# zhang-xuan1314/ABC-Net

Measured on AMD Instinct MI355X. Metric: training images/sec (384x384, b16/GPU), higher is better.
Workload: dtype bf16; 1 GPU; unet.py train step (pack+fwd+fused loss+bwd+allreduce+Adam), 384x384, batch 16/GPU, dropout 0.2; global_batch=16, parallelism=dp1, graph=True, device_meters=False, device_rasteriser=False, device_extraction=False, logits_stored=True

## Files before the change

### abc-net_amd/csrc/bn_act.hip

```cpp
#include "common.hpp"
#include "../../include/abcnet_hip.h"
#include "capi_util.hpp"
#include "reduce_bn.hpp"
#include <stdlib.h>

namespace {

__device__ inline void bn_finalize_fwd_body(const abc_bn_fwd_desc& d, int pstride) {
    __shared__ double sm[4];
    const int c = blockIdx.x;
    if (c >= d.C) return;
    const int rows = d.rows == 4 ? 4 : 2;
    double s1 = 0.0, s2 = 0.0;
    for (int k = threadIdx.x; k < d.nblk; k += 256) {
        s1 += (double)d.partial[((size_t)k * rows + 0) * pstride + c];
        s2 += (double)d.partial[((size_t)k * rows + 1) * pstride + c];
    }
    s1 = block_sum_f64(s1, sm);
    s2 = block_sum_f64(s2, sm);
    if (threadIdx.x == 0) {
        const double mean = s1 / d.count;
        double var = s2 / d.count - mean * mean;
        if (var < 0.0) var = 0.0;
        const float invstd = (float)(1.0 / sqrt(var + (double)d.eps));
        const float sc = d.gamma[c] * invstd;
        d.scale[c] = sc;
        d.shift[c] = d.beta[c] - (float)mean * sc;
        d.mean[c] = (float)mean;
        d.invstd[c] = invstd;
        if (d.running_mean != nullptr) {
            const double unb = d.count > 1.0 ? var * d.count / (d.count - 1.0) : var;
            d.running_mean[c] = (1.f - d.momentum) * d.running_mean[c] + d.momentum * (float)mean;
            d.running_var[c] = (1.f - d.momentum) * d.running_var[c] + d.momentum * (float)unb;
            if (c == 0 && d.num_batches_tracked != nullptr) *d.num_batches_tracked += 1;
        }
    }
}

__global__ __launch_bounds__(256) void bn_finalize_fwd_kernel(const abc_bn_fwd_desc d) { bn_finalize_fwd_body(d, d.C); }
constexpr int MAX_BNB = 8;
struct BnFwdBatch { abc_bn_fwd_desc d[MAX_BNB]; int pstride; };
__global__ __launch_bounds__(256) void bn_finalize_fwd_batch_kernel(const BnFwdBatch bt) {
    bn_finalize_fwd_body(bt.d[blockIdx.y], bt.pstride > 0 ? bt.pstride : bt.d[blockIdx.y].C);
}

__global__ void bn_eval_kernel(const float* gamma, const float* beta, const float* rm, const float* rv, float* scale,
                               float* shift, int C, float eps) {
    const int c = blockIdx.x * blockDim.x + threadIdx.x;
    if (c >= C) return;
    const float sc = gamma[c] / sqrtf(rv[c] + eps);
    scale[c] = sc;
    shift[c] = beta[c] - rm[c] * sc;
}

__global__ void bn_eval_fold_kernel(const float* gamma, const float* beta, const float* rm, const float* rv, const float* cb, float* scale,
                                    float* bias_out, int C, float eps) {
    const int c = blockIdx.x * blockDim.x + threadIdx.x;
    if (c >= C) return;
    const float sc = gamma[c] / sqrtf(rv[c] + eps);
    scale[c] = sc;
    bias_out[c] = ((cb ? cb[c] : 0.f) - rm[c]) * sc + beta[c];
}

__global__ __launch_bounds__(256) void bn_finalize_bwd_kernel(const abc_bn_bwd_desc d) { bn_finalize_bwd_body(d, d.C, blockIdx.x); }
struct BnBwdBatch { abc_bn_bwd_desc d[MAX_BNB]; int pstride; };
__global__ __launch_bounds__(256) void bn_finalize_bwd_batch_kernel(const BnBwdBatch bt) {
    bn_finalize_bwd_body(bt.d[blockIdx.y], bt.pstride > 0 ? bt.pstride : bt.d[blockIdx.y].C, blockIdx.x);
}

template <typename T> struct VecOf;
template <> struct VecOf<float> { static constexpr int N = 4; };
template <> struct VecOf<bf16> { static constexpr int N = 8; };

template <typename T, int N> __device__ inline void ldv(const T* p, float* v) { LoadVec<T, N>::ld(p, v); }
template <int N> __device__ inline void stv(float* p, const float* v) {
    f32x4 t; t[0] = v[0]; t[1] = v[1]; t[2] = v[2]; t[3] = v[3];
    *(f32x4*)p = t;
}
template <int N> __device__ inline void stv(bf16* p, const float* v) {
    bf16x8 t;
#pragma unroll
    for (int j = 0; j < 8; ++j) t[j] = (bf16)v[j];
    *(bf16x8*)p = t;
}

template <typename T>
__global__ __launch_bounds__(256) void act_bwd_plain_kernel(const abc_act_bwd_desc d) {
    constexpr int N = VecOf<T>::N;
    __shared__ float red[256][2 * N + 1];
    const int ncv = d.C / N;
    const unsigned nitems = (unsigned)((int64_t)d.B * d.H * d.W * ncv);
    const unsigned stride = gridDim.x * 256u;
    const int tid = threadIdx.x;
    const int cv = (int)((blockIdx.x * 256 + tid) % ncv);
    const int c = cv * N;
    const int lg = 31 - __builtin_clz((unsigned)ncv);
    float sc[N], sh[N], sl[N], mu[N];
#pragma unroll
    for (int j = 0; j < N; ++j) { sc[j] = d.scale[c + j]; sh[j] = d.shift[c + j]; sl[j] = d.slope[c + j]; mu[j] = d.mean[c + j]; }
    float a1[N], a2[N];
#pragma unroll
    for (int j = 0; j < N; ++j) { a1[j] = 0.f; a2[j] = 0.f; }
    const T* yr = (const T*)d.y_raw + d.cy_off + c;
    const T* ds = (const T*)d.dA_same + d.csame_off + c;
    T* g = (T*)d.g + c;
    auto one = [&](const float* x, const float* da, size_t p) {
        float out[N];
#pragma unroll
        for (int j = 0; j < N; ++j) {
            const float y = fmaf(x[j], sc[j], sh[j]);
            const float gg = y > 0.f ? da[j] : sl[j] * da[j];
            out[j] = gg;
            a1[j] += gg;
            a2[j] = fmaf(gg, x[j] - mu[j], a2[j]);
        }
        stv<N>(g + p * d.ld_g, out);
    };
    unsigned it = blockIdx.x * 256u + tid;
    for (; it + stride < nitems; it += 2 * stride) {
        const size_t p0 = it >> lg, p1 = (it + stride) >> lg;
        float x0[N], d0[N], x1[N], d1[N];
        ldv<T, N>(yr + p0 * d.ld_y, x0); ldv<T, N>(ds + p0 * d.ld_same, d0);
        ldv<T, N>(yr + p1 * d.ld_y, x1); ldv<T, N>(ds + p1 * d.ld_same, d1);
        one(x0, d0, p0);
        one(x1, d1, p1);
    }
    if (it < nitems) {
        const size_t p0 = it >> lg;
        float x0[N], d0[N];
        ldv<T, N>(yr + p0 * d.ld_y, x0); ldv<T, N>(ds + p0 * d.ld_same, d0);
        one(x0, d0, p0);
    }
#pragma unroll
    for (int j = 0; j < N; ++j) { red[tid][j] = a1[j]; red[tid][N + j] = a2[j]; }
    __syncthreads();
    for (int cc = tid; cc < d.C; cc += 256) {
        const int v = cc / N, j = cc % N;
        float s1 = 0.f, s2 = 0.f;
        for (int t = v; t < 256; t += ncv) { s1 += red[t][j]; s2 += red[t][N + j]; }
        d.partial[((size_t)blockIdx.x * 2 + 0) * d.C + cc] = s1;
        d.partial[((size_t)blockIdx.x * 2 + 1) * d.C + cc] = s2 * d.invstd[cc];
    }
}

template <typename T>
__global__ __launch_bounds__(256) void act_bwd_kernel(const abc_act_bwd_desc d) {
    constexpr int N = VecOf<T>::N;
    __shared__ float red[256][2 * N + 1];
    const int ncv = d.C / N;
    const bool pooled = d.dA_pool != nullptr;
    const int Hw = pooled ? d.H / 2 : d.H, Ww = pooled ? d.W / 2 : d.W;
    const int64_t nitems = (int64_t)d.B * Hw * Ww * ncv;
    const int64_t stride = (int64_t)gridDim.x * 256;
    const int tid = threadIdx.x;
    const int cv = (int)((blockIdx.x * 256 + tid) % ncv);
    const int c = cv * N;
    float sc[N], sh[N], sl[N], mu[N], is[N];
#pragma unroll
    for (int j = 0; j < N; ++j) {
        sc[j] = d.scale[c + j]; sh[j] = d.shift[c + j]; sl[j] = d.slope[c + j]; mu[j] = d.mean[c + j]; is[j] = d.invstd[c + j];
    }
    float a1[N], a2[N];
#pragma unroll
    for (int j = 0; j < N; ++j) { a1[j] = 0.f; a2[j] = 0.f; }
    const T* yr = (const T*)d.y_raw;
    const T* ds = (const T*)d.dA_same;
    const T* dp = (const T*)d.dA_pool;
    T* g = (T*)d.g;
    const float dscale = d.drop_p > 0.f ? 1.f / (1.f - d.drop_p) : 1.f;
    const uint32_t dseed = d.drop_seed + ((d.drop_p > 0.f && d.drop_salt) ? *d.drop_salt : 0u);

    const bool pow2 = (ncv & (ncv - 1)) == 0;
    const int lg = 31 - __builtin_clz((unsigned)ncv);
    const unsigned n32 = (unsigned)nitems, st32 = (unsigned)stride;
    for (unsigned it = blockIdx.x * 256u + tid; it < n32; it += st32) {
        unsigned pix = pow2 ? (it >> lg) : (it / (unsigned)ncv);
        if (!pooled) {
            const size_t p = pix;
            float x[N], da[N], out[N];
            ldv<T, N>(yr + p * d.ld_y + d.cy_off + c, x);
            ldv<T, N>(ds + p * d.ld_same + d.csame_off + c, da);
#pragma unroll
            for (int j = 0; j < N; ++j) {
                const float y = fmaf(x[j], sc[j], sh[j]);
                float gg = da[j] * (y > 0.f ? 1.f : sl[j]);
                if (d.drop_p > 0.f)
                    gg = abc_drop_keep((uint32_t)(p * d.drop_ld + d.cy_off + c + j), dseed, d.drop_p) ? gg * dscale : 0.f;
                out[j] = gg;
                a1[j] += gg;
                a2[j] += gg * ((x[j] - mu[j]) * is[j]);
            }
            stv<N>(g + p * d.ld_g + c, out);
        } else {
            const int wx = (int)(pix % (unsigned)Ww); pix /= (unsigned)Ww;
            const int wy = (int)(pix % (unsigned)Hw);
            const int b = (int)(pix / (unsigned)Hw);
            float x[4][N], dpool[N];
            size_t pq[4];
#pragma unroll
            for (int q = 0; q < 4; ++q) {
                pq[q] = ((size_t)b * d.H + 2 * wy + (q >> 1)) * d.W + 2 * wx + (q & 1);
                ldv<T, N>(yr + pq[q] * d.ld_y + d.cy_off + c, x[q]);
            }
            ldv<T, N>(dp + (((size_t)b * Hw + wy) * Ww + wx) * d.ld_pool + d.cpool_off + c, dpool);
            int arg[N];
            float yv[4][N];
#pragma unroll
            for (int j = 0; j < N; ++j) {
                float best = 0.f;
                arg[j] = 0;
#pragma unroll
                for (int q = 0; q < 4; ++q) {
                    const float y = fmaf(x[q][j], sc[j], sh[j]);
                    yv[q][j] = y;
                    const float av = fmaxf(y, sl[j] * y);
                    if (q == 0 || av > best) { best = av; arg[j] = q; }
                }
            }
#pragma unroll
            for (int q = 0; q < 4; ++q) {
                float da[N], out[N];
                if (ds != nullptr) ldv<T, N>(ds + pq[q] * d.ld_same + d.csame_off + c, da);
#pragma unroll
                for (int j = 0; j < N; ++j) {
                    float up = (arg[j] == q) ? dpool[j] : 0.f;
                    if (ds != nullptr) up += da[j];
                    const float gg = up * (yv[q][j] > 0.f ? 1.f : sl[j]);
                    out[j] = gg;
                    a1[j] += gg;
                    a2[j] += gg * ((x[q][j] - mu[j]) * is[j]);
                }
                stv<N>(g + pq[q] * d.ld_g + c, out);
            }
        }
    }
    if (pooled && ((d.H | d.W) & 1)) {
        const int wodd = d.W & 1, hodd = d.H & 1;
        const int ncol = wodd ? d.H : 0;
        const int nrow = hodd ? 2 * Ww : 0;
        const unsigned nl = (unsigned)(ncol + nrow);
        const unsigned n2 = (unsigned)d.B * nl * (unsigned)ncv;
        for (unsigned it = blockIdx.x * 256u + tid; it < n2; it += st32) {
            unsigned l = pow2 ? (it >> lg) : (it / (unsigned)ncv);
            const int b = (int)(l / nl);
            l -= (unsigned)b * nl;
            const int y = (int)l < ncol ? (int)l : d.H - 1, x = (int)l < ncol ? d.W - 1 : (int)l - ncol;
            const size_t p = ((size_t)b * d.H + y) * d.W + x;
            float xv[N], da[N], out[N];
            ldv<T, N>(yr + p * d.ld_y + d.cy_off + c, xv);
            if (ds != nullptr) ldv<T, N>(ds + p * d.ld_same + d.csame_off + c, da);
#pragma unroll
            for (int j = 0; j < N; ++j) {
                const float yv = fmaf(xv[j], sc[j], sh[j]);
                const float gg = (ds != nullptr ? da[j] : 0.f) * (yv > 0.f ? 1.f : sl[j]);
                out[j] = gg;
                a1[j] += gg;
                a2[j] += gg * ((xv[j] - mu[j]) * is[j]);
            }
            stv<N>(g + p * d.ld_g + c, out);
        }
    }
#pragma unroll
    for (int j = 0; j < N; ++j) { red[tid][j] = a1[j]; red[tid][N + j] = a2[j]; }
    __syncthreads();
    for (int cc = tid; cc < d.C; cc += 256) {
        const int v = cc / N, j = cc % N;
        float s1 = 0.f, s2 = 0.f;
        for (int t = v; t < 256; t += ncv) { s1 += red[t][j]; s2 += red[t][N + j]; }
        d.partial[((size_t)blockIdx.x * 2 + 0) * d.C + cc] = s1;
        d.partial[((size_t)blockIdx.x * 2 + 1) * d.C + cc] = s2;
    }
}

template <typename T>
__global__ __launch_bounds__(256) void bn_apply_kernel(const abc_bn_apply_desc d) {
    constexpr int N = VecOf<T>::N;
    const int ncv = d.C / N;
    const int64_t nitems = d.npix * ncv;
    const int64_t stride = (int64_t)gridDim.x * 256;
    T* g = (T*)d.g;
    T* o = d.out ? (T*)d.out : g;
    const int ld_o = d.out ? d.ld_out : d.ld_g;
    const T* yr = (const T*)d.y_raw;
    for (int64_t it = (int64_t)blockIdx.x * 256 + threadIdx.x; it < nitems; it += stride) {
        const int64_t p = it / ncv;
        const int c = (int)(it % ncv) * N;
        float gv[N], x[N], out[N];
        ldv<T, N>(g + p * d.ld_g + c, gv);
        ldv<T, N>(yr + p * d.ld_y + d.cy_off + c, x);
#pragma unroll
        for (int j = 0; j < N; ++j) {
            const float xh = (x[j] - d.mean[c + j]) * d.invstd[c + j];
            out[j] = d.gscale[c + j] * (gv[j] - d.k1[c + j] - xh * d.k2[c + j]);
        }
        stv<N>(o + p * ld_o + c, out);
    }
}
// ... 84 lines not shown
    const T* base = x + c_off + cv * N;
    int64_t p = (int64_t)blockIdx.x * PL + pl;
    const int64_t step = (int64_t)gridDim.x * PL;
    for (; p + 3 * step < npix; p += 4 * step) {
        float a[4][N], wv[4];
#pragma unroll
        for (int u = 0; u < 4; ++u) { ldv<T, N>(base + (p + u * step) * ld, a[u]); wv[u] = w[p + u * step]; }
#pragma unroll
        for (int u = 0; u < 4; ++u)
#pragma unroll
            for (int j = 0; j < N; ++j) { acc[j] += a[u][j]; accw[j] = fmaf(a[u][j], wv[u], accw[j]); }
    }
    for (; p < npix; p += step) {
        float a[N];
        ldv<T, N>(base + p * ld, a);
        const float wv = w[p];
#pragma unroll
        for (int j = 0; j < N; ++j) { acc[j] += a[j]; accw[j] = fmaf(a[j], wv, accw[j]); }
    }
#pragma unroll
    for (int j = 0; j < N; ++j) { red[threadIdx.x][j] = acc[j]; red[threadIdx.x][N + j] = accw[j]; }
    __syncthreads();
    for (int c = threadIdx.x; c < 2 * C; c += 256) {
        const int row = c / C, cc = c - row * C;
        const int v = cc / N, j = cc % N;
        float s = 0.f;
        for (int q = 0; q < PL; ++q) s += red[q * ncv + v][row * N + j];
        work[((size_t)blockIdx.x * 2 + row) * C + cc] = s;
    }
}
__global__ __launch_bounds__(256) void colsum_w1_reduce_kernel(const float* work, int nblk, int C, float* out_sum, float* out_w) {
    __shared__ double sm[4];
    const int c = blockIdx.x, row = blockIdx.y;
    double s = 0.0;
    for (int k = threadIdx.x; k < nblk; k += 256) s += (double)work[((size_t)k * 2 + row) * C + c];
    s = block_sum_f64(s, sm);
    if (threadIdx.x == 0) {
        if (row == 0) { if (out_sum != nullptr) out_sum[c] = (float)s; }
        else out_w[c] = (float)s;
    }
}

__global__ void fill_kernel(float* p, float v, int64_t n) {
    for (int64_t i = (int64_t)blockIdx.x * blockDim.x + threadIdx.x; i < n; i += (int64_t)gridDim.x * blockDim.x) p[i] = v;
}

__global__ __launch_bounds__(256) void nhwc_to_nchw_kernel(const float* src, int ld, int c_off, int C, int HW, float* dst) {
    __shared__ float tile[32][33];
    const int b = blockIdx.z;
    const int p0 = blockIdx.x * 32, c0 = blockIdx.y * 32;
    const int tx = threadIdx.x & 31, ty = threadIdx.x >> 5;
    for (int k = ty; k < 32; k += 8) {
        const int p = p0 + k, c = c0 + tx;
        tile[k][tx] = (p < HW && c < C) ? src[((size_t)b * HW + p) * ld + c_off + c] : 0.f;
    }
    __syncthreads();
    for (int k = ty; k < 32; k += 8) {
        const int c = c0 + k, p = p0 + tx;
        if (p < HW && c < C) dst[((size_t)b * C + c) * HW + p] = tile[tx][k];
    }
}
__global__ __launch_bounds__(256) void nchw_to_nhwc_kernel(const float* src, int C, int HW, float* dst, int ld, int c_off) {
    __shared__ float tile[32][33];
    const int b = blockIdx.z;
    const int p0 = blockIdx.x * 32, c0 = blockIdx.y * 32;
    const int tx = threadIdx.x & 31, ty = threadIdx.x >> 5;
    for (int k = ty; k < 32; k += 8) {
        const int c = c0 + k, p = p0 + tx;
        tile[k][tx] = (p < HW && c < C) ? src[((size_t)b * C + c) * HW + p] : 0.f;
    }
    __syncthreads();
    for (int k = ty; k < 32; k += 8) {
        const int p = p0 + k, c = c0 + tx;
        if (p < HW && c < C) dst[((size_t)b * HW + p) * ld + c_off + c] = tile[tx][k];
    }
}

static int ew_blocks(int64_t nitems) {
    int64_t b = (nitems + 255) / 256;
    if (b > 2048) b = 2048;
    if (b < 1) b = 1;
    return (int)b;
}

}

extern "C" int abc_bn_finalize_fwd(const abc_bn_fwd_desc* d, abc_stream_t stream) {
    if (d->C < 1 || d->nblk < 1) return abc_fail(ABC_EINVAL, "bn_finalize_fwd: empty");
    hipLaunchKernelGGL(bn_finalize_fwd_kernel, dim3(d->C), dim3(256), 0, (hipStream_t)stream, *d);
    return abc_check_launch("bn_finalize_fwd");
}

extern "C" int abc_bn_finalize_fwd_batch(const abc_bn_fwd_desc* descs, int32_t n, int32_t pstride, abc_stream_t stream) {
    if (n < 1 || n > MAX_BNB) return abc_fail(ABC_EINVAL, "bn_finalize_fwd_batch: 1..8 layers");
    BnFwdBatch bt;
    int cmax = 0;
    for (int i = 0; i < n; ++i) { bt.d[i] = descs[i]; cmax = descs[i].C > cmax ? descs[i].C : cmax; if (descs[i].C < 1 || descs[i].nblk < 1) return abc_fail(ABC_EINVAL, "bn_finalize_fwd_batch: empty"); }
    for (int i = n; i < MAX_BNB; ++i) bt.d[i] = descs[0];
    bt.pstride = pstride;
    hipLaunchKernelGGL(bn_finalize_fwd_batch_kernel, dim3(cmax, n), dim3(256), 0, (hipStream_t)stream, bt);
    return abc_check_launch("bn_finalize_fwd_batch");
}

extern "C" int abc_bn_finalize_bwd_batch(const abc_bn_bwd_desc* descs, int32_t n, int32_t pstride, abc_stream_t stream) {
    if (n < 1 || n > MAX_BNB) return abc_fail(ABC_EINVAL, "bn_finalize_bwd_batch: 1..8 layers");
    BnBwdBatch bt;
    int cmax = 0;
    for (int i = 0; i < n; ++i) { bt.d[i] = descs[i]; cmax = descs[i].C > cmax ? descs[i].C : cmax; if (descs[i].C < 1 || descs[i].nblk < 1) return abc_fail(ABC_EINVAL, "bn_finalize_bwd_batch: empty"); }
    for (int i = n; i < MAX_BNB; ++i) bt.d[i] = descs[0];
    bt.pstride = pstride;
    hipLaunchKernelGGL(bn_finalize_bwd_batch_kernel, dim3(cmax, n), dim3(256), 0, (hipStream_t)stream, bt);
    return abc_check_launch("bn_finalize_bwd_batch");
}

extern "C" int abc_bn_eval_coeffs(const float* gamma, const float* beta, const float* running_mean, const float* running_var,
                                  float* scale, float* shift, int32_t C, float eps, abc_stream_t stream) {
    hipLaunchKernelGGL(bn_eval_kernel, dim3(abc_cdiv(C, 256)), dim3(256), 0, (hipStream_t)stream, gamma, beta, running_mean,
                       running_var, scale, shift, C, eps);
    return abc_check_launch("bn_eval_coeffs");
}

extern "C" int abc_bn_eval_fold(const float* gamma, const float* beta, const float* running_mean, const float* running_var,
                                const float* conv_bias, float* scale, float* bias_out, int32_t C, float eps, abc_stream_t stream) {
    hipLaunchKernelGGL(bn_eval_fold_kernel, dim3(abc_cdiv(C, 256)), dim3(256), 0, (hipStream_t)stream, gamma, beta, running_mean,
                       running_var, conv_bias, scale, bias_out, C, eps);
    return abc_check_launch("bn_eval_fold");
}

extern "C" int abc_bn_finalize_bwd(const abc_bn_bwd_desc* d, abc_stream_t stream) {
    if (d->C < 1 || d->nblk < 1) return abc_fail(ABC_EINVAL, "bn_finalize_bwd: empty");
    hipLaunchKernelGGL(bn_finalize_bwd_kernel, dim3(d->C), dim3(256), 0, (hipStream_t)stream, *d);
    return abc_check_launch("bn_finalize_bwd");
}

static int act_bwd_check(const abc_act_bwd_desc* d) {
    const int N = d->dtype == ABC_BF16 ? 8 : 4;
    if (d->C % N) return abc_fail(ABC_EINVAL, "act_bwd: C must be a multiple of the vector width");
    const int ncv = d->C / N;
    if (ncv > 256 || (256 % ncv)) return abc_fail(ABC_EUNSUPPORTED, "act_bwd: C/vec must divide 256");
    if (d->dA_pool && (((d->H | d->W) & 1) && d->drop_p > 0.f)) return abc_fail(ABC_EUNSUPPORTED, "act_bwd: odd pooled dims with dropout");
    if (!d->dA_pool && !d->dA_same) return abc_fail(ABC_EINVAL, "act_bwd: no gradient source");
    if ((d->ld_y | d->ld_g | d->cy_off) % N) return abc_fail(ABC_EINVAL, "act_bwd: alignment");
    if ((int64_t)d->B * d->H * d->W * ncv >= (int64_t(1) << 31)) return abc_fail(ABC_EUNSUPPORTED, "act_bwd: tensor too large for 32-bit indexing");
    return ABC_OK;
}

extern "C" int abc_act_bwd_blocks(const abc_act_bwd_desc* d) {
    const int N = d->dtype == ABC_BF16 ? 8 : 4;
    const bool pooled = d->dA_pool != nullptr;
    const int64_t n = (int64_t)d->B * (pooled ? d->H / 2 : d->H) * (pooled ? d->W / 2 : d->W) * (d->C / N);
    return ew_blocks(n);
}

extern "C" int abc_act_bwd(const abc_act_bwd_desc* d, abc_stream_t stream) {
    int rc = act_bwd_check(d);
    if (rc) return rc;
    const int nb = abc_act_bwd_blocks(d);
    if (d->dA_pool == nullptr && d->drop_p <= 0.f) {
        if (d->dtype == ABC_BF16) hipLaunchKernelGGL(act_bwd_plain_kernel<bf16>, dim3(nb), dim3(256), 0, (hipStream_t)stream, *d);
        else hipLaunchKernelGGL(act_bwd_plain_kernel<float>, dim3(nb), dim3(256), 0, (hipStream_t)stream, *d);
        return abc_check_launch("act_bwd");
    }
    if (d->dtype == ABC_BF16) hipLaunchKernelGGL(act_bwd_kernel<bf16>, dim3(nb), dim3(256), 0, (hipStream_t)stream, *d);
    else hipLaunchKernelGGL(act_bwd_kernel<float>, dim3(nb), dim3(256), 0, (hipStream_t)stream, *d);
    return abc_check_launch("act_bwd");
}

extern "C" int abc_bn_apply_bwd(const abc_bn_apply_desc* d, abc_stream_t stream) {
    const int N = d->dtype == ABC_BF16 ? 8 : 4;
    if (d->C % N || (d->ld_g | d->ld_y | d->cy_off) % N || (d->out && d->ld_out % N)) return abc_fail(ABC_EINVAL, "bn_apply: alignment");
    const int nb = ew_blocks(d->npix * (d->C / N));
    if (d->dtype == ABC_BF16) hipLaunchKernelGGL(bn_apply_kernel<bf16>, dim3(nb), dim3(256), 0, (hipStream_t)stream, *d);
    else hipLaunchKernelGGL(bn_apply_kernel<float>, dim3(nb), dim3(256), 0, (hipStream_t)stream, *d);
    return abc_check_launch("bn_apply_bwd");
}

extern "C" int abc_colsum_blocks(int64_t npix) {
    int64_t b = (npix + 63) / 64;
    return (int)(b < 1 ? 1 : (b > 1024 ? 1024 : b));
}

extern "C" int abc_colsum(const void* x, int32_t dtype, int64_t npix, int32_t ld, int32_t c_off, int32_t C,
                          const float* chan_scale, float* work, float* out, abc_stream_t stream) {
    const int nb = abc_colsum_blocks(npix);
    hipStream_t st = (hipStream_t)stream;
    if (C > 512) return abc_fail(ABC_EUNSUPPORTED, "colsum: C > 512");
    {
        const int N = dtype == ABC_BF16 ? 8 : 4;
        const int ncv = C / N;
        if (C % N == 0 && ncv >= 1 && ncv <= 256 && 256 % ncv == 0 && ld % N == 0 && c_off % N == 0) {
            if (dtype == ABC_BF16)
                hipLaunchKernelGGL(colsum_vec_kernel<bf16>, dim3(nb), dim3(256), 0, st, (const bf16*)x, npix, ld, c_off, C, chan_scale, work);
            else
                hipLaunchKernelGGL(colsum_vec_kernel<float>, dim3(nb), dim3(256), 0, st, (const float*)x, npix, ld, c_off, C, chan_scale, work);
            hipLaunchKernelGGL(colsum_reduce_kernel, dim3(C), dim3(256), 0, st, (const float*)work, nb, C, out);
            return abc_check_launch("colsum");
        }
    }
    int CW = 1;
    while (CW < C && CW < 64) CW <<= 1;
    if (dtype == ABC_BF16)
        hipLaunchKernelGGL(colsum_kernel<bf16>, dim3(nb), dim3(256), 0, st, (const bf16*)x, npix, ld, c_off, C, chan_scale, work, CW);
    else
        hipLaunchKernelGGL(colsum_kernel<float>, dim3(nb), dim3(256), 0, st, (const float*)x, npix, ld, c_off, C, chan_scale, work, CW);
    hipLaunchKernelGGL(colsum_reduce_kernel, dim3(C), dim3(256), 0, st, (const float*)work, nb, C, out);
    return abc_check_launch("colsum");
}

extern "C" int abc_colsum_w1(const void* x, int32_t dtype, int64_t npix, int32_t ld, int32_t c_off, int32_t C, const float* w,
                             float* work, float* out_sum, float* out_w, abc_stream_t stream) {
    const int nb = abc_colsum_blocks(npix);
    const int N = dtype == ABC_BF16 ? 8 : 4;
    const int ncv = C / N;
    if (x == nullptr || w == nullptr || work == nullptr || out_w == nullptr) return abc_fail(ABC_EINVAL, "colsum_w1: x, w, work and out_w are required");
    if (C % N || ncv < 1 || ncv > 256 || 256 % ncv || ld % N || c_off % N)
        return abc_fail(ABC_EUNSUPPORTED, "colsum_w1: C / vector width must divide 256, ld and c_off be multiples of the vector width");
    hipStream_t st = (hipStream_t)stream;
    if (dtype == ABC_BF16) hipLaunchKernelGGL(colsum_w1_kernel<bf16>, dim3(nb), dim3(256), 0, st, (const bf16*)x, npix, ld, c_off, C, w, work);
    else hipLaunchKernelGGL(colsum_w1_kernel<float>, dim3(nb), dim3(256), 0, st, (const float*)x, npix, ld, c_off, C, w, work);
    hipLaunchKernelGGL(colsum_w1_reduce_kernel, dim3(C, 2), dim3(256), 0, st, (const float*)work, nb, C, out_sum, out_w);
    return abc_check_launch("colsum_w1");
}

template <typename InT, typename OutT>
__global__ __launch_bounds__(256) void pool_act_kernel(const InT* x, const float* sc, const float* sh, const float* sl, int Hx, int Wx,
                                                        int ldx, int c_off, int C, int64_t nseg, OutT* out, int ld_out) {
    const int64_t i = (int64_t)blockIdx.x * 256 + threadIdx.x;
    if (i >= nseg) return;
    const int segs = C / 8;
    const int sg = (int)(i % segs);
    int64_t pix = i / segs;
    const int Wo = Wx / 2, Ho = Hx / 2;
    const int xo = (int)(pix % Wo); pix /= Wo;
    const int yo = (int)(pix % Ho);
    const int b = (int)(pix / Ho);
    const int c = c_off + sg * 8;
    float a[8], s_[8], t_[8];
    const bool tr = sc != nullptr;
#pragma unroll
    for (int j = 0; j < 8; ++j) { a[j] = tr ? sc[c + j] : 1.f; s_[j] = tr ? sh[c + j] : 0.f; t_[j] = tr ? sl[c + j] : 1.f; }
    float m[8];
#pragma unroll
    for (int q = 0; q < 4; ++q) {
        float v[8];
        LoadVec<InT, 8>::ld(x + ((size_t)(b * Hx + 2 * yo + (q >> 1)) * Wx + 2 * xo + (q & 1)) * ldx + c, v);
#pragma unroll
        for (int j = 0; j < 8; ++j) {
            const float y = tr ? abc_act(v[j], a[j], s_[j], t_[j]) : v[j];
            m[j] = (q == 0) ? y : fmaxf(m[j], y);
        }
    }
    OutT* dst = out + ((size_t)(b * Ho + yo) * Wo + xo) * ld_out + sg * 8;
    if constexpr (sizeof(OutT) == 2) {
        *(bf16x8*)dst = pack_frag<bf16>(m);
    } else {
        f32x4 lo, hi;
#pragma unroll
        for (int j = 0; j < 4; ++j) { lo[j] = m[j]; hi[j] = m[4 + j]; }
        *(f32x4*)dst = lo; *(f32x4*)(dst + 4) = hi;
    }
}

extern "C" int abc_pool_act(const abc_act_src* src, int32_t dtype_in, int32_t c_off, int32_t C, int32_t B, void* out, int32_t dtype_out,
                            int32_t ld_out, abc_stream_t stream) {
    if (C % 8 || c_off % 8 || src->ldx % 8 || ld_out % 8 || src->Hx < 2 || src->Wx < 2) return abc_fail(ABC_EINVAL, "pool_act: alignment");
    if (src->planar || src->drop_p > 0.f) return abc_fail(ABC_EUNSUPPORTED, "pool_act: planar / dropout source");
    const int64_t nseg = (int64_t)B * (src->Hx / 2) * (src->Wx / 2) * (C / 8);
    const dim3 grid((unsigned)((nseg + 255) / 256));
    hipStream_t st = (hipStream_t)stream;
    if (dtype_in == ABC_BF16 && dtype_out == ABC_BF16)
        hipLaunchKernelGGL((pool_act_kernel<bf16, bf16>), grid, dim3(256), 0, st, (const bf16*)src->x, src->scale, src->shift, src->slope, src->Hx,
                           src->Wx, src->ldx, c_off, C, nseg, (bf16*)out, ld_out);
    else if (dtype_in == ABC_F32 && dtype_out == ABC_F32)
        hipLaunchKernelGGL((pool_act_kernel<float, float>), grid, dim3(256), 0, st, (const float*)src->x, src->scale, src->shift, src->slope,
                           src->Hx, src->Wx, src->ldx, c_off, C, nseg, (float*)out, ld_out);
    else if (dtype_in == ABC_F32 && dtype_out == ABC_BF16)
        hipLaunchKernelGGL((pool_act_kernel<float, bf16>), grid, dim3(256), 0, st, (const float*)src->x, src->scale, src->shift, src->slope,
                           src->Hx, src->Wx, src->ldx, c_off, C, nseg, (bf16*)out, ld_out);
    else return abc_fail(ABC_EUNSUPPORTED, "pool_act: dtype combination");
    return abc_check_launch("pool_act");
}

extern "C" int abc_fill_f32(float* p, float v, int64_t n, abc_stream_t stream) {
    if (n <= 0) return ABC_OK;
    hipLaunchKernelGGL(fill_kernel, dim3(ew_blocks(n)), dim3(256), 0, (hipStream_t)stream, p, v, n);
    return abc_check_launch("fill");
}

extern "C" int abc_nhwc_to_nchw_f32(const float* src, int32_t ld, int32_t c_off, int32_t C, int32_t B, int32_t H, int32_t W,
                                    float* dst, abc_stream_t stream) {
    const int HW = H * W;
    hipLaunchKernelGGL(nhwc_to_nchw_kernel, dim3(abc_cdiv(HW, 32), abc_cdiv(C, 32), B), dim3(256), 0, (hipStream_t)stream, src,
                       ld, c_off, C, HW, dst);
    return abc_check_launch("nhwc_to_nchw");
}

extern "C" int abc_nchw_to_nhwc_f32(const float* src, int32_t C, int32_t B, int32_t H, int32_t W, float* dst, int32_t ld,
                                    int32_t c_off, abc_stream_t stream) {
    const int HW = H * W;
    hipLaunchKernelGGL(nchw_to_nhwc_kernel, dim3(abc_cdiv(HW, 32), abc_cdiv(C, 32), B), dim3(256), 0, (hipStream_t)stream, src,
                       C, HW, dst, ld, c_off);
    return abc_check_launch("nchw_to_nhwc");
}
```

### abc-net_amd/csrc/misc.hip

```cpp
#include "common.hpp"
#include "../../include/abcnet_hip.h"
#include "capi_util.hpp"
#include <string.h>

static thread_local char g_err[256] = "";
int abc_fail(int code, const char* msg) {
    strncpy(g_err, msg, sizeof(g_err) - 1);
    g_err[sizeof(g_err) - 1] = 0;
    return code;
}
int abc_allow_lds(const void* fn, int bytes, unsigned long long* done) {
    int dev = 0;
    if (hipGetDevice(&dev) != hipSuccess) dev = -1;
    if (dev >= 0 && dev < 64 && ((*done >> dev) & 1ull)) return ABC_OK;
    hipError_t e = hipFuncSetAttribute(fn, hipFuncAttributeMaxDynamicSharedMemorySize, bytes);
    if (e != hipSuccess) {
        snprintf(g_err, sizeof(g_err), "hipFuncSetAttribute(MaxDynamicSharedMemorySize=%d) on device %d: %s", bytes, dev, hipGetErrorString(e));
        return ABC_ELAUNCH;
    }
    if (dev >= 0 && dev < 64) *done |= 1ull << dev;
    return ABC_OK;
}
int abc_check_launch(const char* what) {
    hipError_t e = hipGetLastError();
    if (e != hipSuccess) {
        snprintf(g_err, sizeof(g_err), "%s: %s", what, hipGetErrorString(e));
        return ABC_ELAUNCH;
    }
    return ABC_OK;
}
extern "C" const char* abc_last_error(void) { return g_err; }
extern "C" int abc_version(void) { return 101; }
extern "C" int abc_set_reserved_cus(int n) {
    if (n < 0 || n > 128) return abc_fail(ABC_EINVAL, "abc_set_reserved_cus: 0 <= n <= 128");
    abc_reserved_cus_ref() = (n + 3) & ~3;
    return ABC_OK;
}
extern "C" int abc_get_reserved_cus(void) { return abc_reserved_cus_ref(); }

namespace {

__host__ __device__ inline size_t abc_pack_offset(size_t slice, int rows, int row, int CK, int k, int layout) {
    if (layout == 1) {
        const int sh = CK == 64 ? 4 : 3;
        const int h = k >> (sh + 1), kk = (k >> sh) & 1, e = k & ((1 << sh) - 1);
        return (slice * rows + (size_t)(row & ~31)) * CK + (size_t)((((kk * 2 + h) * 32 + (row & 31)) << sh) + e);
    }
    return (slice * rows + row) * CK + k;
}

template <typename CT>
__global__ void pack_kernel(const abc_pack_desc d, int CK, int ntaps, int nchunks) {
    const int nch_total = (d.red_total + CK - 1) / CK, ch_off = d.red_off / CK;
    const int64_t total = (int64_t)ntaps * nchunks * d.rows_pad * CK;
    CT* dst = (CT*)d.dst;
    for (int64_t i = (int64_t)blockIdx.x * blockDim.x + threadIdx.x; i < total; i += (int64_t)gridDim.x * blockDim.x) {
        const int k = (int)(i % CK);
        int64_t r = i / CK;
        const int n = (int)(r % d.rows_pad); r /= d.rows_pad;
        const int c = (int)(r % nchunks);
        const int t = (int)(r / nchunks);
        const int rc = c * CK + k;
        float v = 0.f;
        if (d.mode == 0) {
            if (n < d.Cout && rc < d.Cin) v = d.w[((size_t)n * d.Cin + rc) * ntaps + t];
        } else if (d.mode == 1) {
            if (n < d.Cin && rc < d.Cout) v = d.w[((size_t)rc * d.Cin + n) * ntaps + t];
        } else if (d.mode == 2) {
            const int nx = d.px ? 2 : 1;
            const int iy = t / nx, ix = t % nx;
            const int ky = d.py ? (iy == 0 ? 0 : 2) : 1;
            const int kx = d.px ? (ix == 0 ? 0 : 2) : 1;
            if (n < d.Cout && rc < d.Cin) v = d.w[(((size_t)rc * d.Cout + n) * 3 + ky) * 3 + kx];
        } else {
            if (n < d.Cin && rc < d.Cout) v = d.w[((size_t)n * d.Cout + rc) * 9 + t];
        }
        if (d.row_scale != nullptr && (d.mode == 0 || d.mode == 2) && n < d.Cout) v *= d.row_scale[n];
        const int rtot = d.rows_total > 0 ? d.rows_total : d.rows_pad;
        dst[abc_pack_offset((size_t)t * nch_total + ch_off + c, rtot, d.rows_off + n, CK, k, d.layout)] = CT(v);
    }
}

struct PackItem { abc_pack_desc d; int32_t CK, ntaps, nchunks, dtype; int64_t first; int32_t ntiles, pad_; };
__device__ inline void pack_one(const PackItem& it, unsigned r) {
    const abc_pack_desc& d = it.d;
    const unsigned CK = it.CK, ntaps = it.ntaps, nchunks = it.nchunks, rows = d.rows_pad;
    const unsigned k = r % CK; r /= CK;
    const unsigned n = r % rows; r /= rows;
    const unsigned c = r % nchunks;
    const unsigned t = r / nchunks;
    const unsigned rc = c * CK + k;
    float v = 0.f;
    if (d.mode == 0) {
        if (n < (unsigned)d.Cout && rc < (unsigned)d.Cin) v = d.w[((size_t)n * d.Cin + rc) * ntaps + t];
    } else if (d.mode == 1) {
        if (n < (unsigned)d.Cin && rc < (unsigned)d.Cout) v = d.w[((size_t)rc * d.Cin + n) * ntaps + t];
    } else if (d.mode == 2) {
        const unsigned nx = d.px ? 2 : 1;
        const unsigned iy = t / nx, ix = t % nx;
        const unsigned ky = d.py ? (iy == 0 ? 0 : 2) : 1;
        const unsigned kx = d.px ? (ix == 0 ? 0 : 2) : 1;
        if (n < (unsigned)d.Cout && rc < (unsigned)d.Cin) v = d.w[(((size_t)rc * d.Cout + n) * 3 + ky) * 3 + kx];
    } else {
        if (n < (unsigned)d.Cin && rc < (unsigned)d.Cout) v = d.w[((size_t)n * d.Cout + rc) * 9 + t];
    }
    if (d.row_scale != nullptr && (d.mode == 0 || d.mode == 2) && n < (unsigned)d.Cout) v *= d.row_scale[n];
    const unsigned nch_total = (d.red_total + CK - 1) / CK, ch_off = d.red_off / CK;
    const unsigned rtot = d.rows_total > 0 ? (unsigned)d.rows_total : rows;
    const size_t o = abc_pack_offset((size_t)t * nch_total + ch_off + c, (int)rtot, (int)((unsigned)d.rows_off + n), (int)CK, (int)k, d.layout);
    if (it.dtype == ABC_BF16) ((bf16*)d.dst)[o] = (bf16)v; else if (it.dtype == ABC_FP8) ((f8*)d.dst)[o] = f8(v); else ((float*)d.dst)[o] = v;
}

constexpr int PACK_CHUNK = 2048;
__device__ inline int pack_find(const PackItem* items, int nitems, int64_t i) {
    int lo = 0, hi = nitems - 1;
    while (lo < hi) {
        const int mid = (lo + hi + 1) >> 1;
        if (items[mid].first <= i) lo = mid; else hi = mid - 1;
    }
    return lo;
}
__global__ __launch_bounds__(256) void pack_batch_kernel(const PackItem* items, int nitems, int64_t total) {
    __shared__ int s_lo, s_hi;
    const int64_t i0 = (int64_t)blockIdx.x * PACK_CHUNK;
    const int64_t i1 = (i0 + PACK_CHUNK < total) ? i0 + PACK_CHUNK : total;
    if (threadIdx.x == 0) { s_lo = pack_find(items, nitems, i0); s_hi = pack_find(items, nitems, i1 - 1); }
    __syncthreads();
    const int lo = __builtin_amdgcn_readfirstlane(s_lo), hi = __builtin_amdgcn_readfirstlane(s_hi);
    if (lo == hi) {
        const PackItem it = items[lo];
        if (it.ntiles > 0) return;
        const unsigned base = (unsigned)(i0 - it.first);
        for (unsigned e = threadIdx.x; e < (unsigned)(i1 - i0); e += 256) pack_one(it, base + e);
    } else {
        for (int64_t i = i0 + threadIdx.x; i < i1; i += 256) {
            const int j = pack_find(items, nitems, i);
            if (items[j].ntiles > 0) continue;
            pack_one(items[j], (unsigned)(i - items[j].first));
        }
    }
}

constexpr int PT_MAXT = 9;
constexpr int PT_MAXITEMS = 1023;
__global__ __launch_bounds__(256) void pack_tiles_kernel(const PackItem* items, int nitems) {
    __shared__ float tile[32 * (32 * PT_MAXT + 1)];
    __shared__ int s_nt[PT_MAXITEMS + 1];
    __shared__ int s_item, s_tile;
    const int tid = threadIdx.x;
    for (int j = tid; j < nitems; j += 256) s_nt[j + 1] = items[j].ntiles;
    __syncthreads();
    if (tid == 0) {
        s_nt[0] = 0;
        for (int j = 0; j < nitems; ++j) s_nt[j + 1] += s_nt[j];
    }
    __syncthreads();
    const int total = s_nt[nitems];
    for (int tg = blockIdx.x; tg < total; tg += gridDim.x) {
        __syncthreads();
        if (tid == 0) {
            int lo = 0, hi = nitems - 1;
            while (lo < hi) { const int mid = (lo + hi + 1) >> 1; if (s_nt[mid] <= tg) lo = mid; else hi = mid - 1; }
            s_item = lo; s_tile = tg - s_nt[lo];
        }
        __syncthreads();
        const PackItem it = items[__builtin_amdgcn_readfirstlane(s_item)];
        const abc_pack_desc& d = it.d;
        const int tl = __builtin_amdgcn_readfirstlane(s_tile);
        const int ntaps = it.ntaps, nchunks = it.nchunks;
        const int c = tl % nchunks, rb = tl / nchunks;
        const int n0 = rb * 32, k0 = c * 32;
        const int S = 32 * ntaps + 1;
        const int rows_real = d.mode == 0 ? d.Cout : d.Cin;
        const bool real = n0 < rows_real;
        if (real) {
            if ((((uintptr_t)d.w) & 15) == 0) {
                const int j = tid >> 3, q0 = tid & 7;
                const float* src = d.mode == 0 ? d.w + ((size_t)(n0 + j) * d.Cin + k0) * ntaps : d.w + ((size_t)(k0 + j) * d.Cin + n0) * ntaps;
                f32x4 v[PT_MAXT];
#pragma unroll
                for (int m = 0; m < PT_MAXT; ++m) {
                    if (m < ntaps) v[m] = *(const f32x4*)(src + 4 * (q0 + 8 * m));
                }
#pragma unroll
                for (int m = 0; m < PT_MAXT; ++m) {
                    if (m < ntaps) {
                        float* o = tile + j * S + 4 * (q0 + 8 * m);
                        o[0] = v[m][0]; o[1] = v[m][1]; o[2] = v[m][2]; o[3] = v[m][3];
                    }
                }
            } else {
                const int wv = tid >> 6, ln = tid & 63;
                constexpr int NQ = (32 * PT_MAXT + 63) / 64;
                float v[8][NQ];
#pragma unroll
                for (int jj = 0; jj < 8; ++jj) {
                    const int j = wv * 8 + jj;
                    const float* src = d.mode == 0 ? d.w + ((size_t)(n0 + j) * d.Cin + k0) * ntaps : d.w + ((size_t)(k0 + j) * d.Cin + n0) * ntaps;
#pragma unroll
                    for (int m = 0; m < NQ; ++m) {
                        const int q = ln + 64 * m;
                        v[jj][m] = q < 32 * ntaps ? src[q] : 0.f;
                    }
                }
#pragma unroll
                for (int jj = 0; jj < 8; ++jj) {
#pragma unroll
                    for (int m = 0; m < NQ; ++m) {
                        const int q = ln + 64 * m;
                        if (q < 32 * ntaps) tile[(wv * 8 + jj) * S + q] = v[jj][m];
                    }
                }
            }
        }
        __syncthreads();
        const int nch_total = (d.red_total + 31) / 32, ch_off = d.red_off / 32;
        const int rtot = d.rows_total > 0 ? d.rows_total : d.rows_pad;
        const int r = tid & 31, g = (tid >> 5) & 3, th = tid >> 7;
        const float rs = (real && d.row_scale != nullptr && d.mode == 0) ? d.row_scale[n0 + r] : 1.f;
        for (int t = th; t < ntaps; t += 2) {
            bf16x8 o;
#pragma unroll
            for (int i = 0; i < 8; ++i) {
                float v = 0.f;
                if (real) v = d.mode == 0 ? tile[r * S + (8 * g + i) * ntaps + t] : tile[(8 * g + i) * S + r * ntaps + t];
                if (d.row_scale != nullptr && d.mode == 0) v *= rs;
                o[i] = (bf16)v;
            }
            const size_t off = abc_pack_offset((size_t)t * nch_total + ch_off + c, rtot, d.rows_off + n0 + r, 32, 8 * g, d.layout);
            *(bf16x8*)((bf16*)d.dst + off) = o;
        }
    }
}

__global__ void step_inc_kernel(int64_t* step) { *step += 1; }

__global__ __launch_bounds__(256) void adam_kernel(const abc_adam_desc d) {
    const double t = (double)*d.step;
    const float bc1 = (float)(1.0 - pow((double)d.beta1, t));
    const float bc2s = (float)sqrt(1.0 - pow((double)d.beta2, t));
    const float step_size = d.lr / bc1;
    const int64_t n4 = d.n / 4;
    const int64_t stride = (int64_t)gridDim.x * 256;
    for (int64_t i = (int64_t)blockIdx.x * 256 + threadIdx.x; i < n4; i += stride) {
        f32x4 p = ((f32x4*)d.p)[i], g = ((const f32x4*)d.g)[i], m = ((f32x4*)d.m)[i], v = ((f32x4*)d.v)[i];
#pragma unroll
        for (int j = 0; j < 4; ++j) {
            const float gg = g[j] * d.grad_scale + d.weight_decay * p[j];
            m[j] = m[j] + (gg - m[j]) * (1.f - d.beta1);
            v[j] = v[j] * d.beta2 + (1.f - d.beta2) * gg * gg;
            p[j] -= step_size * m[j] / (sqrtf(v[j]) / bc2s + d.eps);
        }
        ((f32x4*)d.p)[i] = p; ((f32x4*)d.m)[i] = m; ((f32x4*)d.v)[i] = v;
    }
    if (blockIdx.x == 0) {
        for (int64_t i = n4 * 4 + threadIdx.x; i < d.n; i += 256) {
            const float gg = d.g[i] * d.grad_scale + d.weight_decay * d.p[i];
            const float m = d.m[i] + (gg - d.m[i]) * (1.f - d.beta1);
            const float v = d.v[i] * d.beta2 + (1.f - d.beta2) * gg * gg;
            d.m[i] = m; d.v[i] = v;
            d.p[i] -= step_size * m / (sqrtf(v) / bc2s + d.eps);
        }
    }
}

__global__ __launch_bounds__(256) void nms_kernel(const abc_nms_desc d) {
    const int hw = d.h * d.w;
    const int64_t npix = (int64_t)d.B * hw;
    const int64_t p = (int64_t)blockIdx.x * 256 + threadIdx.x;
    if (p >= npix) return;
    const int b = (int)(p / hw), yx = (int)(p % hw);
    const int y = yx / d.w, x = yx % d.w;
    for (int which = 0; which < 2; ++which) {
        const float* L = (which ? d.bond : d.atom) + (size_t)b * hw;
        const float v = L[yx];
        float m = v;
        for (int dy = -1; dy <= 1; ++dy)
            for (int dx = -1; dx <= 1; ++dx) {
                const int yy = y + dy, xx = x + dx;
                if (yy >= 0 && yy < d.h && xx >= 0 && xx < d.w) m = fmaxf(m, L[yy * d.w + xx]);
            }
        float* o = which ? d.bond_mask : d.atom_mask;
        o[(size_t)b * hw + yx] = (m == v && v > -1.f) ? 1.f : 0.f;
    }
    const int n = d.n_omega;
    if (n <= 0) return;
    const float* R = d.rho + (size_t)b * n * hw + yx;
    const float* O = d.omega + (size_t)b * n * hw + yx;
    float prev = O[(size_t)(n - 1) * hw], cur = O[0];
    const float first = cur;
    for (int k = 0; k < n; ++k) {
// ... 270 lines not shown
```

Before: 2885 images/sec.

## Add specialised pooled act-backward kernel and vectorise bf16 weight packing

Adds a bf16 act-backward kernel for the max-pool case without dropout. It processes whole 2x2 windows with 32-bit indexing and a magic-number divide, and has SAME/no-SAME variants with different occupancy hints. The weight pack kernel now finds item ranges with a parallel scan instead of a per-element binary search, and writes eight bf16 values per thread in a vector store when alignment allows. pool_act gets 32-bit index math and vectorised parameter loads. The aim is to cut integer-division and scattered-store overhead, at the cost of more code paths and possible small numeric-ordering differences from the contract-off accumulation.

```diff
diff --git a/abc-net_amd/csrc/bn_act.hip b/abc-net_amd/csrc/bn_act.hip
--- a/abc-net_amd/csrc/bn_act.hip
+++ b/abc-net_amd/csrc/bn_act.hip
@@ -143,6 +143,102 @@
     }
 }
 
+__device__ inline void ldc8(const float* p, float* v) {
+    if ((((uintptr_t)p) & 15) == 0) {
+        const f32x4 lo = *(const f32x4*)p, hi = *(const f32x4*)(p + 4);
+#pragma unroll
+        for (int j = 0; j < 4; ++j) { v[j] = lo[j]; v[4 + j] = hi[j]; }
+    } else {
+#pragma unroll
+        for (int j = 0; j < 8; ++j) v[j] = p[j];
+    }
+}
+
+template <bool SAME>
+__device__ inline void pool_window_bwd(const bf16x8 (&x)[4], const bf16x8& dpool, const bf16x8 (&da)[4], const float* sc, const float* sh,
+                                       const float* sl, const float* mu, const float* is, float* a1, float* a2, bf16x8 (&out)[4]) {
+#pragma clang fp contract(off)
+#pragma unroll
+    for (int j = 0; j < 8; ++j) {
+        float xv[4], yv[4];
+        float best = 0.f;
+        int arg = 0;
+#pragma unroll
+        for (int q = 0; q < 4; ++q) {
+            xv[q] = (float)x[q][j];
+            const float y = __builtin_fmaf(xv[q], sc[j], sh[j]);
+            yv[q] = y;
+            const float av = fmaxf(y, sl[j] * y);
+            if (q == 0 || av > best) { best = av; arg = q; }
+        }
+        const float dpv = (float)dpool[j];
+#pragma unroll
+        for (int q = 0; q < 4; ++q) {
+            float up = (arg == q) ? dpv : 0.f;
+            if (SAME) up = (float)da[q][j] + up;
+            const float dact = yv[q] > 0.f ? 1.f : sl[j];
+            const float gg = up * dact;
+            out[q][j] = (bf16)gg;
+            a1[j] = q < 3 ? a1[j] + gg : __builtin_fmaf(up, dact, a1[j]);
+            a2[j] = __builtin_fmaf(gg, (xv[q] - mu[j]) * is[j], a2[j]);
+        }
+        asm volatile("" : "+v"(a1[j]), "+v"(a2[j]));
+    }
+}
+
+template <bool SAME, int WAVES>
+__global__ __launch_bounds__(256, WAVES) void act_bwd_pool_kernel(const abc_act_bwd_desc d, const unsigned magic) {
+    constexpr int N = 8;
+    __shared__ float red[256][2 * N + 1];
+    const int ncv = d.C / N;
+    const unsigned Ww = (unsigned)d.W / 2u;
+    const unsigned nitems = (unsigned)d.B * ((unsigned)d.H / 2u) * Ww * (unsigned)ncv;
+    const unsigned stride = gridDim.x * 256u;
+    const int tid = threadIdx.x;
+    const int cv = (int)((blockIdx.x * 256 + tid) % ncv);
+    const int c = cv * N;
+    const int lg = 31 - __builtin_clz((unsigned)ncv);
+    float sc[N], sh[N], sl[N], mu[N], is[N];
+#pragma unroll
+    for (int j = 0; j < N; ++j) {
+        sc[j] = d.scale[c + j]; sh[j] = d.shift[c + j]; sl[j] = d.slope[c + j]; mu[j] = d.mean[c + j]; is[j] = d.invstd[c + j];
+    }
+    float a1[N], a2[N];
+#pragma unroll
+    for (int j = 0; j < N; ++j) { a1[j] = 0.f; a2[j] = 0.f; }
+    const bf16* yr = (const bf16*)d.y_raw + d.cy_off + c;
+    const bf16* ds = SAME ? (const bf16*)d.dA_same + d.csame_off + c : nullptr;
+    const bf16* dp = (const bf16*)d.dA_pool + d.cpool_off + c;
+    bf16* g = (bf16*)d.g + c;
+    const unsigned W = (unsigned)d.W;
+    for (unsigned it = blockIdx.x * 256u + tid; it < nitems; it += stride) {
+        const unsigned pix = it >> lg;
+        const unsigned row = __umulhi(pix, magic);
+        const unsigned p0 = 4u * row * Ww + 2u * (pix - row * Ww);
+        bf16x8 x[4], dpool, da[4], out[4];
+#pragma unroll
+        for (int q = 0; q < 4; ++q) x[q] = *(const bf16x8*)(yr + (p0 + (q >> 1) * W + (q & 1)) * (unsigned)d.ld_y);
+        dpool = *(const bf16x8*)(dp + pix * (unsigned)d.ld_pool);
+        if (SAME) {
+#pragma unroll
+            for (int q = 0; q < 4; ++q) da[q] = *(const bf16x8*)(ds + (p0 + (q >> 1) * W + (q & 1)) * (unsigned)d.ld_same);
+        }
+        pool_window_bwd<SAME>(x, dpool, da, sc, sh, sl, mu, is, a1, a2, out);
+#pragma unroll
+        for (int q = 0; q < 4; ++q) *(bf16x8*)(g + (p0 + (q >> 1) * W + (q & 1)) * (unsigned)d.ld_g) = out[q];
+    }
+#pragma unroll
+    for (int j = 0; j < N; ++j) { red[tid][j] = a1[j]; red[tid][N + j] = a2[j]; }
+    __syncthreads();
+    for (int cc = tid; cc < d.C; cc += 256) {
+        const int v = cc / N, j = cc % N;
+        float s1 = 0.f, s2 = 0.f;
+        for (int t = v; t < 256; t += ncv) { s1 += red[t][j]; s2 += red[t][N + j]; }
+        d.partial[((size_t)blockIdx.x * 2 + 0) * d.C + cc] = s1;
+        d.partial[((size_t)blockIdx.x * 2 + 1) * d.C + cc] = s2;
+    }
+}
+
 template <typename T>
 __global__ __launch_bounds__(256) void act_bwd_kernel(const abc_act_bwd_desc d) {
     constexpr int N = VecOf<T>::N;
@@ -533,6 +629,15 @@
     return ew_blocks(n);
 }
 
+static bool act_bwd_pool_fast(const abc_act_bwd_desc* d) {
+    if (d->dtype != ABC_BF16 || d->dA_pool == nullptr || d->drop_p > 0.f || ((d->H | d->W) & 1) || d->W < 4) return false;
+    const int64_t npix = (int64_t)d->B * d->H * d->W, npool = npix / 4;
+    int ld = d->ld_y > d->ld_g ? d->ld_y : d->ld_g;
+    if (d->dA_same != nullptr && d->ld_same > ld) ld = d->ld_same;
+    if (ld < 1 || d->ld_pool < 1 || npix * ld >= (int64_t(1) << 31) || npool * d->ld_pool >= (int64_t(1) << 31)) return false;
+    return npool * (d->W / 2) < (int64_t(1) << 32);
+}
+
 extern "C" int abc_act_bwd(const abc_act_bwd_desc* d, abc_stream_t stream) {
     int rc = act_bwd_check(d);
     if (rc) return rc;
@@ -540,6 +645,14 @@
     if (d->dA_pool == nullptr && d->drop_p <= 0.f) {
         if (d->dtype == ABC_BF16) hipLaunchKernelGGL(act_bwd_plain_kernel<bf16>, dim3(nb), dim3(256), 0, (hipStream_t)stream, *d);
         else hipLaunchKernelGGL(act_bwd_plain_kernel<float>, dim3(nb), dim3(256), 0, (hipStream_t)stream, *d);
+        return abc_check_launch("act_bwd");
+    }
+    if (act_bwd_pool_fast(d)) {
+        const unsigned magic = (unsigned)(((uint64_t(1) << 32) + (uint64_t)(d->W / 2) - 1) / (uint64_t)(d->W / 2));
+        const bool same = d->dA_same != nullptr;
+        hipStream_t st = (hipStream_t)stream;
+        if (same) hipLaunchKernelGGL((act_bwd_pool_kernel<true, 3>), dim3(nb), dim3(256), 0, st, *d, magic);
+        else hipLaunchKernelGGL((act_bwd_pool_kernel<false, 4>), dim3(nb), dim3(256), 0, st, *d, magic);
         return abc_check_launch("act_bwd");
     }
     if (d->dtype == ABC_BF16) hipLaunchKernelGGL(act_bwd_kernel<bf16>, dim3(nb), dim3(256), 0, (hipStream_t)stream, *d);
@@ -609,17 +722,30 @@
     const int64_t i = (int64_t)blockIdx.x * 256 + threadIdx.x;
     if (i >= nseg) return;
     const int segs = C / 8;
-    const int sg = (int)(i % segs);
-    int64_t pix = i / segs;
     const int Wo = Wx / 2, Ho = Hx / 2;
-    const int xo = (int)(pix % Wo); pix /= Wo;
-    const int yo = (int)(pix % Ho);
-    const int b = (int)(pix / Ho);
+    int sg, xo, yo, b;
+    if (nseg < (int64_t(1) << 31)) {
+        unsigned u = (unsigned)i;
+        sg = (int)(u % (unsigned)segs); u /= (unsigned)segs;
+        xo = (int)(u % (unsigned)Wo); u /= (unsigned)Wo;
+        yo = (int)(u % (unsigned)Ho);
+        b = (int)(u / (unsigned)Ho);
+    } else {
+        sg = (int)(i % segs);
+        int64_t pix = i / segs;
+        xo = (int)(pix % Wo); pix /= Wo;
+        yo = (int)(pix % Ho);
+        b = (int)(pix / Ho);
+    }
     const int c = c_off + sg * 8;
     float a[8], s_[8], t_[8];
     const bool tr = sc != nullptr;
-#pragma unroll
-    for (int j = 0; j < 8; ++j) { a[j] = tr ? sc[c + j] : 1.f; s_[j] = tr ? sh[c + j] : 0.f; t_[j] = tr ? sl[c + j] : 1.f; }
+    if (tr) {
+        ldc8(sc + c, a); ldc8(sh + c, s_); ldc8(sl + c, t_);
+    } else {
+#pragma unroll
+        for (int j = 0; j < 8; ++j) { a[j] = 1.f; s_[j] = 0.f; t_[j] = 1.f; }
+    }
     float m[8];
 #pragma unroll
     for (int q = 0; q < 4; ++q) {
diff --git a/abc-net_amd/csrc/misc.hip b/abc-net_amd/csrc/misc.hip
--- a/abc-net_amd/csrc/misc.hip
+++ b/abc-net_amd/csrc/misc.hip
@@ -111,32 +111,68 @@
     if (it.dtype == ABC_BF16) ((bf16*)d.dst)[o] = (bf16)v; else if (it.dtype == ABC_FP8) ((f8*)d.dst)[o] = f8(v); else ((float*)d.dst)[o] = v;
 }
 
+__device__ inline void pack_eight_bf16(const PackItem& it, unsigned r) {
+    const abc_pack_desc& d = it.d;
+    const unsigned CK = it.CK, ntaps = it.ntaps, nchunks = it.nchunks, rows = d.rows_pad;
+    const unsigned lgck = 31 - __builtin_clz(CK);
+    const unsigned k0 = r & (CK - 1); r >>= lgck;
+    const unsigned n = r % rows; r /= rows;
+    const unsigned c = r % nchunks;
+    const unsigned t = r / nchunks;
+    const unsigned rc0 = c * CK + k0;
+    unsigned base, step, rowlim, redlim;
+    if (d.mode == 0) {
+        base = (n * d.Cin + rc0) * ntaps + t; step = ntaps; rowlim = d.Cout; redlim = d.Cin;
+    } else if (d.mode == 1) {
+        base = (rc0 * d.Cin + n) * ntaps + t; step = d.Cin * ntaps; rowlim = d.Cin; redlim = d.Cout;
+    } else if (d.mode == 2) {
+        const unsigned nx = d.px ? 2 : 1;
+        const unsigned iy = t / nx, ix = t % nx;
+        const unsigned ky = d.py ? (iy == 0 ? 0 : 2) : 1;
+        const unsigned kx = d.px ? (ix == 0 ? 0 : 2) : 1;
+        base = ((rc0 * d.Cout + n) * 3 + ky) * 3 + kx; step = d.Cout * 9; rowlim = d.Cout; redlim = d.Cin;
+    } else {
+        base = (n * d.Cout + rc0) * 9 + t; step = 9; rowlim = d.Cin; redlim = d.Cout;
+    }
+    float v[8];
+#pragma unroll
+    for (int i = 0; i < 8; ++i) v[i] = (n < rowlim && rc0 + i < redlim) ? d.w[base + i * step] : 0.f;
+    if (d.row_scale != nullptr && (d.mode == 0 || d.mode == 2) && n < (unsigned)d.Cout) {
+        const float rs = d.row_scale[n];
+#pragma unroll
+        for (int i = 0; i < 8; ++i) v[i] *= rs;
+    }
+    const unsigned nch_total = (d.red_total + CK - 1) >> lgck, ch_off = (unsigned)d.red_off >> lgck;
+    const unsigned rtot = d.rows_total > 0 ? (unsigned)d.rows_total : rows;
+    const size_t o = abc_pack_offset((size_t)t * nch_total + ch_off + c, (int)rtot, (int)((unsigned)d.rows_off + n), (int)CK, (int)k0, d.layout);
+    bf16x8 ov;
+#pragma unroll
+    for (int i = 0; i < 8; ++i) ov[i] = (bf16)v[i];
+    *(bf16x8*)((bf16*)d.dst + o) = ov;
+}
+
 constexpr int PACK_CHUNK = 2048;
-__device__ inline int pack_find(const PackItem* items, int nitems, int64_t i) {
-    int lo = 0, hi = nitems - 1;
-    while (lo < hi) {
-        const int mid = (lo + hi + 1) >> 1;
-        if (items[mid].first <= i) lo = mid; else hi = mid - 1;
-    }
-    return lo;
-}
 __global__ __launch_bounds__(256) void pack_batch_kernel(const PackItem* items, int nitems, int64_t total) {
     __shared__ int s_lo, s_hi;
     const int64_t i0 = (int64_t)blockIdx.x * PACK_CHUNK;
     const int64_t i1 = (i0 + PACK_CHUNK < total) ? i0 + PACK_CHUNK : total;
-    if (threadIdx.x == 0) { s_lo = pack_find(items, nitems, i0); s_hi = pack_find(items, nitems, i1 - 1); }
+    for (int j = threadIdx.x; j < nitems; j += 256) {
+        const int64_t f = items[j].first, e = j + 1 < nitems ? items[j + 1].first : total;
+        if (f <= i0 && i0 < e) s_lo = j;
+        if (f < i1 && i1 <= e) s_hi = j;
+    }
     __syncthreads();
     const int lo = __builtin_amdgcn_readfirstlane(s_lo), hi = __builtin_amdgcn_readfirstlane(s_hi);
-    if (lo == hi) {
-        const PackItem it = items[lo];
-        if (it.ntiles > 0) return;
-        const unsigned base = (unsigned)(i0 - it.first);
-        for (unsigned e = threadIdx.x; e < (unsigned)(i1 - i0); e += 256) pack_one(it, base + e);
-    } else {
-        for (int64_t i = i0 + threadIdx.x; i < i1; i += 256) {
-            const int j = pack_find(items, nitems, i);
-            if (items[j].ntiles > 0) continue;
-            pack_one(items[j], (unsigned)(i - items[j].first));
+    for (int j = lo; j <= hi; ++j) {
+        const PackItem it = items[j];
+        const int64_t end = j + 1 < nitems ? items[j + 1].first : total;
+        const int64_t a = it.first > i0 ? it.first : i0, b = end < i1 ? end : i1;
+        if (it.ntiles > 0 || a >= b) continue;
+        const unsigned base = (unsigned)(a - it.first), cnt = (unsigned)(b - a);
+        if (it.dtype == ABC_BF16 && ((base | cnt | (unsigned)it.CK) & 7u) == 0 && (((uintptr_t)it.d.dst) & 15) == 0) {
+            for (unsigned e = threadIdx.x * 8u; e < cnt; e += 2048u) pack_eight_bf16(it, base + e);
+        } else {
+            for (unsigned e = threadIdx.x; e < cnt; e += 256) pack_one(it, base + e);
         }
     }
 }
```

Result: faster. 2922 images/sec, median of 6 (+1.3%).
